# DoubangoTelecom/compv

Measured on AMD Instinct MI355X. Metric: Mpixels/s Sobel->Canny->HoughSHT on 4K uint8, higher is better.
Workload: dtype u8; 1 GPU; batched 3840x2160 uint8 frames, Sobel3x3 -> Canny(59,119) -> HoughSHT(rho=1, theta=1deg, thr=100); 256 distinct frames resident per GPU as 8 batches of 32, a step processes one batch, steps rotate over the batches; frames_per_gpu=32, resident_batches=8, parallelism=frames sharded across 1 GPU(s), no data-path collective

## Files before the change

### compv_amd/csrc/api.cpp

```cpp
#include "api_internal.hpp"

namespace {
__attribute__((noinline, optnone)) float libmCosf(float x) { return cosf(x); }
__attribute__((noinline, optnone)) float libmSinf(float x) { return sinf(x); }

void gradientThresholds(float fLow, float fHigh, int* tLow, int* tHigh)
{
	const float l = fLow < 1.f ? 1.f : (fLow > 65535.f ? 65535.f : fLow);
	const float h = fHigh < 1.f ? 1.f : (fHigh > 65535.f ? 65535.f : fHigh);
	uint16_t lo = static_cast<uint16_t>(l), hi = static_cast<uint16_t>(h);
	lo = static_cast<uint16_t>(std::max<int>(1, lo));
	hi = static_cast<uint16_t>(std::max<int>(lo + 2, hi));
	*tLow = lo; *tHigh = hi;
}

void cannyCoverage(size_t W, int* simdEnd, int* cStart)
{
	const size_t maxCols = W - 1;
	size_t mpw = 1;
	if (maxCols >= 16) mpw = 16; else if (maxCols >= 8) mpw = 8;
	if (mpw == 1) { *simdEnd = 1; *cStart = 1; return; }
	size_t col = 1;
	while (col + (mpw - 1) < maxCols) col += mpw;
	*simdEnd = static_cast<int>(col);
// ... 218 lines not shown
	HIPCHK(ctx, dmalloc(ctx, &p->sinQ, T));
	HIPCHK(ctx, dmalloc(ctx, &p->cosQ, T));
	HIPCHK(ctx, hipMemcpy(p->sinQ, s.data(), T * sizeof(int32_t), hipMemcpyHostToDevice));
	HIPCHK(ctx, hipMemcpy(p->cosQ, c.data(), T * sizeof(int32_t), hipMemcpyHostToDevice));
	{
		std::vector<float> ct(T), ist(T);
		for (size_t t = 0; t < T; ++t) {
			const float theta = static_cast<float>(t) * step;
			ct[t] = libmCosf(theta);
			ist[t] = 1.f / libmSinf(theta);
		}
		HIPCHK(ctx, dmalloc(ctx, &p->cosT, T));
		HIPCHK(ctx, dmalloc(ctx, &p->invSinT, T));
		HIPCHK(ctx, hipMemcpy(p->cosT, ct.data(), T * sizeof(float), hipMemcpyHostToDevice));
		HIPCHK(ctx, hipMemcpy(p->invSinT, ist.data(), T * sizeof(float), hipMemcpyHostToDevice));
	}
	{
		if (p->vt.tiles <= 0 || p->vtKt.size() != static_cast<size_t>(p->vt.tiles) * T) return fail(ctx, COMPVHIP_E_INVALID_STATE, "vote tiles were not planned");
		dfree(ctx, p->dKt); dfree(ctx, p->dRowBase); dfree(ctx, p->partLo); dfree(ctx, p->partHi); dfree(ctx, p->colFlag);
		{
			const int tiles = p->vt.tiles, Rw = p->vt.Rw, groups = sht_nms_groups(static_cast<int>(T));
			std::vector<int2> range(static_cast<size_t>(groups));
			for (int g = 0; g < groups; ++g) {
				int lo = INT32_MAX, hi = INT32_MIN;
				for (int c = 8 * g - 1; c <= 8 * g + 8; ++c) {
					if (c < 0 || c >= static_cast<int>(T)) continue;
					for (int i = 0; i < tiles; ++i) {
						const int b = p->vtRowBase[static_cast<size_t>(i) * T + c];
						lo = std::min(lo, b); hi = std::max(hi, b + Rw);
					}
				}
				range[g] = make_int2(lo - 1, hi + 1);
			}
			std::vector<int2> reach(T);
			for (size_t t = 0; t < T; ++t) {
				int lo = INT32_MAX, hi = INT32_MIN;
				for (int i = 0; i < tiles; ++i) {
					const int b = p->vtRowBase[static_cast<size_t>(i) * T + t];
					lo = std::min(lo, b); hi = std::max(hi, b + Rw);
				}
				reach[t] = make_int2(lo, hi);
			}
			dfree(ctx, p->reach);
			HIPCHK(ctx, dmalloc(ctx, &p->reach, reach.size()));
			HIPCHK(ctx, hipMemcpy(p->reach, reach.data(), reach.size() * sizeof(int2), hipMemcpyHostToDevice));
			dfree(ctx, p->nmsRange);
			HIPCHK(ctx, dmalloc(ctx, &p->nmsRange, range.size()));
			HIPCHK(ctx, hipMemcpy(p->nmsRange, range.data(), range.size() * sizeof(int2), hipMemcpyHostToDevice));
		}
		HIPCHK(ctx, dmalloc(ctx, &p->dKt, p->vtKt.size()));
		HIPCHK(ctx, dmalloc(ctx, &p->dRowBase, p->vtRowBase.size()));
		HIPCHK(ctx, hipMemcpy(p->dKt, p->vtKt.data(), p->vtKt.size() * sizeof(int32_t), hipMemcpyHostToDevice));
		HIPCHK(ctx, hipMemcpy(p->dRowBase, p->vtRowBase.data(), p->vtRowBase.size() * sizeof(int32_t), hipMemcpyHostToDevice));
		{
			const size_t cols = p->frames * p->vt.tiles * static_cast<size_t>(p->vt.Tpad);
			HIPCHK(ctx, dmalloc(ctx, &p->partLo, cols * p->vt.rwPitch));
			HIPCHK(ctx, dmalloc(ctx, &p->partHi, cols * p->vt.rwPitch));
			HIPCHK(ctx, dmalloc(ctx, &p->colFlag, cols));
		}
		p->vt.kt = p->dKt; p->vt.rowBase = p->dRowBase; p->vt.partLo = p->partLo; p->vt.partHi = p->partHi; p->vt.colFlag = p->colFlag; p->vt.reach = p->reach; p->vt.tileCounts = p->tileCounts;
		p->edgeCap = static_cast<size_t>(p->vt.tiles) * p->vt.tileCap;
	}
	HIPCHK(ctx, dmalloc(ctx, &p->edges, p->edgeCap * p->frames));
	HIPCHK(ctx, dmalloc(ctx, &p->acc, p->accFrameStride * p->frames));
	HIPCHK(ctx, hipMemset(p->acc, 0, sizeof(uint16_t) * p->accFrameStride * p->frames));
	p->strengthBits = 1;
	while ((static_cast<size_t>(1) << p->strengthBits) <= 2 * (p->W > p->H ? p->W : p->H)) p->strengthBits++;
	if (p->strengthBits > 16) p->strengthBits = 16;
	int frameBits = 0;
	while ((static_cast<size_t>(1) << frameBits) < p->frames) frameBits++;
	p->keyBits = frameBits + p->strengthBits;
	if (R * T >= (static_cast<size_t>(1) << 32)) return fail(ctx, COMPVHIP_E_INVALID_PARAMETER, "theta step too small: the accumulator has 2^32 cells or more");
	if (p->keyBits > 32) return fail(ctx, COMPVHIP_E_INVALID_PARAMETER, "too many frames for a 32-bit line key");
	dfree(ctx, p->nmsFlags);
	{
		const size_t frows = sht_nms_rows(static_cast<int>(R)), fgroups = static_cast<size_t>(sht_nms_groups(static_cast<int>(T)));
		HIPCHK(ctx, dmalloc(ctx, &p->nmsFlags, frows * fgroups * p->frames));
		HIPCHK(ctx, hipMemset(p->nmsFlags, 0, frows * fgroups * p->frames));
		if (sht_lines_blocks(static_cast<int>(R)) != p->lineBlocks) return fail(ctx, COMPVHIP_E_INVALID_STATE, "row-block counters were sized for another accumulator");
	}
	p->shtReady = true;
	return COMPVHIP_OK;
}

int compvhip_api::ensureLineCap(compvhip_plan* p, size_t cap)
{
	compvhip_ctx* ctx = p->ctx;
	cap = std::min(cap, p->R * p->T);
	if (cap <= p->lineCap) return COMPVHIP_OK;
	dfree(ctx, p->keysA); dfree(ctx, p->keysB); dfree(ctx, p->valsA); dfree(ctx, p->valsB); dfree(ctx, p->sortTemp); dfree(ctx, p->chunkHist); dfree(ctx, p->strengthStart);
	p->lineCap = 0; p->deviceSort = false;
	HIPCHK(ctx, dmalloc(ctx, &p->keysA, cap * p->frames));
	HIPCHK(ctx, dmalloc(ctx, &p->keysB, cap * p->frames));
// ... 183 lines not shown
		if (dmalloc(ctx, &p->sums, frames * kFrameSlot) != hipSuccess) { rc = COMPVHIP_E_OUT_OF_MEMORY; break; }
		if (hipHostMalloc(reinterpret_cast<void**>(&p->hFlags), sizeof(int) * 2 * (kAsyncDepth + 1)) != hipSuccess) { rc = COMPVHIP_E_OUT_OF_MEMORY; break; }
		p->hTotals = reinterpret_cast<unsigned int*>(p->hFlags + kAsyncDepth + 1);
		if (hipHostMalloc(reinterpret_cast<void**>(&p->hRounds), sizeof(int) * (kFrameSlot + 4) * kAsyncDepth, hipHostMallocMapped) != hipSuccess) { rc = COMPVHIP_E_OUT_OF_MEMORY; break; }
		if (hipHostGetDevicePointer(reinterpret_cast<void**>(&p->hRoundsDev), p->hRounds, 0) != hipSuccess) { rc = COMPVHIP_E_HIP; break; }
	} while (0);
	if (rc) { compvhip_plan_destroy(p); return fail(ctx, rc, "plan allocation"); }
	*out = p;
	return COMPVHIP_OK;
}

void compvhip_plan_destroy(compvhip_plan* p)
{
	if (!p) return;
	compvhip_ctx* ctx = p->ctx;
	(void)hipSetDevice(ctx->device);
	timelineClear(p);
	for (hipEvent_t e : p->eventPool) (void)hipEventDestroy(e);
	for (auto& stp : p->steps) if (stp.done) (void)hipEventDestroy(stp.done);
	dfree(ctx, p->dirty);
	dfree(ctx, p->ebits); dfree(ctx, p->ubits); dfree(ctx, p->counters); dfree(ctx, p->thrDev); dfree(ctx, p->sums); dfree(ctx, p->tmpOut);
	if (p->hFlags) (void)hipHostFree(p->hFlags);
	if (p->hRounds) (void)hipHostFree(p->hRounds);
	dfree(ctx, p->hist); dfree(ctx, p->otsu); dfree(ctx, p->blurTmp); dfree(ctx, p->grayTmp);
	dfree(ctx, p->morphTmp);
	dfree(ctx, p->fastWork); dfree(ctx, p->fastScores);
	p->orbIndex.release(ctx); dfree(ctx, p->orbBlur);
	for (KhtBatchState* b : p->khtBatch) khtBatchFree(ctx, b);
	p->khtBatch.clear();
	dfree(ctx, p->cosT); dfree(ctx, p->invSinT);
	dfree(ctx, p->dKt); dfree(ctx, p->dRowBase); dfree(ctx, p->partLo); dfree(ctx, p->partHi); dfree(ctx, p->colFlag);
	dfree(ctx, p->sinQ); dfree(ctx, p->cosQ); dfree(ctx, p->edges); dfree(ctx, p->acc);
	dfree(ctx, p->keysA); dfree(ctx, p->keysB); dfree(ctx, p->valsA); dfree(ctx, p->valsB); dfree(ctx, p->nmsFlags); dfree(ctx, p->chunkHist); dfree(ctx, p->strengthStart);
	dfree(ctx, p->nmsRange); dfree(ctx, p->reach); dfree(ctx, p->sortTemp); p->segPerLine.release(ctx);
	dfree(ctx, p->compRows); dfree(ctx, p->compBits); dfree(ctx, p->compParent);
	delete p;
}

int compvhip_plan_set_timing(compvhip_plan* p, int enabled)
{
	if (!p) return COMPVHIP_E_INVALID_PARAMETER;
	p->timing = (enabled >= 2 && enabled <= 4) ? enabled : (enabled != 0 ? 1 : 0);
	return COMPVHIP_OK;
}

int compvhip_plan_get_timing(compvhip_plan* p, const char** names, float* ms, int cap)
{
	if (!p) return COMPVHIP_E_INVALID_PARAMETER;
	(void)hipSetDevice(p->ctx->device);
	if (!p->timeline.empty()) {
		for (auto& t : p->timeline) (void)hipEventSynchronize(t.b);
		timelineCollect(p);
	}
	const int n = std::min<int>(cap, static_cast<int>(p->timingMs.size()));
	for (int i = 0; i < n; ++i) { if (names) names[i] = p->timingNames[i].c_str(); if (ms) ms[i] = p->timingMs[i]; }
	return n;
}

static int planCannyImpl(compvhip_plan* p, const uint8_t* d_in, float tLow, float tHigh, int ksize, int type, uint8_t* d_edges, hipStream_t st,
                         bool waitConverged, bool clearTimeline = true)
{
	compvhip_ctx* ctx = p->ctx;
	if (!d_in || !d_edges) return fail(ctx, COMPVHIP_E_INVALID_PARAMETER, "null frame pointer");
	int lo, hi;
	int rc = validateCannyParams(ctx, tLow, tHigh, ksize, type, &lo, &hi);
	if (rc) return rc;
	HIPCHK(ctx, hipSetDevice(ctx->device));
// ... 435 lines not shown
```

### compv_amd/csrc/api_internal.hpp

```cpp
#pragma once
#include "../../include/compv_hip.h"
#include "kernels.hpp"
#include "kht.hpp"

#include <hip/hip_runtime.h>

#include <algorithm>
#include <atomic>
#include <chrono>
#include <cmath>
#include <cstdio>
#include <cstdlib>
#include <cstring>
#include <functional>
#include <memory>
#include <string>
#include <thread>
#include <vector>

using namespace compvhip;

namespace compvhip_api {
void countLive(compvhip_ctx* ctx, long delta);

// ... 147 lines not shown
	compvhip_ctx* ctx = nullptr;
	size_t W = 0, H = 0, S = 0, frames = 0;
	float thetaDeg = 1.f;
	int tilesX = 0, tilesY = 0, wb = 0;
	size_t bitsFrameStride = 0;
	uint32_t* ebits = nullptr; uint32_t* ubits = nullptr;
	int* counters = nullptr;
	size_t nCounts = 0;
	int* flags = nullptr; int* hFlags = nullptr;
	int* frameTotals = nullptr; unsigned int* lineTotal = nullptr;
	unsigned int* hTotals = nullptr;
	unsigned int recentTotals[8] = {}; int recentN = 0;
	int specRounds = kSpecRounds; unsigned char recentRounds[8] = {}; int recentRoundsN = 0;
	int* hRoundsDev = nullptr; int* stepHostSlot = nullptr;
	int* hRounds = nullptr;
	int roundsUsed = 0;
	int maxRounds = kMaxRounds;
	bool countersFresh = false;
	int2* thrDev = nullptr; unsigned int* sums = nullptr;
	uint8_t* dirty = nullptr;
	uint8_t* patchOut = nullptr; uint8_t* copyBack = nullptr;
	uint8_t* grayTmp = nullptr;
	uint8_t* tmpOut = nullptr;
	bool bitsValid = false;
	bool shtReady = false;
	size_t R = 0, T = 0; float thetaStep = 0.f; int accPitch = 0;
	uint8_t* blurTmp = nullptr;
	uint32_t* hist = nullptr; int32_t* otsu = nullptr;
	float* cosT = nullptr; float* invSinT = nullptr;
	int32_t* sinQ = nullptr; int32_t* cosQ = nullptr;
	uint32_t* edges = nullptr; size_t edgeCap = 0; int* edgeCounts = nullptr;
	uint16_t* acc = nullptr; size_t accFrameStride = 0;
	uint32_t* keysA = nullptr; uint32_t* keysB = nullptr; uint32_t* valsA = nullptr; uint32_t* valsB = nullptr; size_t lineCap = 0; int* lineCounts = nullptr;
	int2* reach = nullptr;
	int2* nmsRange = nullptr;
	uint8_t* nmsFlags = nullptr;
	int* blockCounts = nullptr; int lineBlocks = 0;
	void* sortTemp = nullptr; size_t sortTempBytes = 0;
	DevBuf<int32_t> segPerLine;
	int32_t* compRows = nullptr; uint32_t* compBits = nullptr; int32_t* compParent = nullptr;
	uint8_t* morphTmp = nullptr;
	int* fastWork = nullptr; uint8_t* fastScores = nullptr;
	DevBuf<int32_t> orbIndex; uint8_t* orbBlur = nullptr; uint16_t orbKern[5] = {}; bool orbKernReady = false; bool orbBriefLds = false;
	int strengthBits = 16, keyBits = 0;
	uint16_t* chunkHist = nullptr; uint32_t* strengthStart = nullptr; int sortChunks = 0; bool deviceSort = false;
	bool voteTiles = false;
	ShtTileArgs vt = {};
	std::vector<int32_t> vtKt, vtRowBase;
	int32_t* dKt = nullptr; int32_t* dRowBase = nullptr; uint8_t* partLo = nullptr; uint8_t* partHi = nullptr; uint8_t* colFlag = nullptr; int* tileCounts = nullptr;
	std::vector<KhtBatchState*> khtBatch;
	std::vector<std::unique_ptr<KhtPeaksWork>> khtWork;
	double khtStageMs[6] = {}; double khtWallMs = 0.0; int khtThreads = 0;
	struct AsyncStep { bool used = false; bool replay = false; uint64_t seq = 0; hipEvent_t done = nullptr; hipStream_t stream = nullptr; StepParams sp; size_t sortN = 0; int rounds = 0; } steps[kAsyncDepth];
	uint64_t stepSeq = 0;
};

struct compvhip_matcher : TimingState {
	compvhip_ctx* ctx = nullptr;
	int descDwords = 0, queryCap = 0, trainCap = 0, pairs = 0, knn = 0;
	uint32_t* partial = nullptr;
	compvhip_match* reverse = nullptr;
};
namespace compvhip_api {

inline void countLive(compvhip_ctx* ctx, long delta) { ctx->live += delta; }

inline int fail(compvhip_ctx* ctx, int code, const char* what, hipError_t e = hipSuccess)
// ... 90 lines not shown
```

### compv_amd/csrc/kernels.hpp

```cpp
#pragma once
#include <hip/hip_runtime.h>
#include <stddef.h>
#include <stdint.h>

#include "../../include/compv_hip.h"

namespace compvhip {

#ifndef COMPVHIP_BAND_H
#define COMPVHIP_BAND_H 64
#endif
constexpr int kBandH = COMPVHIP_BAND_H;
#ifndef COMPVHIP_BAND_WORDS
#define COMPVHIP_BAND_WORDS 64
#endif
constexpr int kBandWords = COMPVHIP_BAND_WORDS;
constexpr int kResolveThreads = 512;
constexpr int kFrameSlot = 32;
constexpr int kResolveRows = kBandH * kBandWords / kResolveThreads;

struct CannyArgs {
	const uint8_t* in;
	uint8_t* out;
	uint32_t* ebits;
// ... 74 lines not shown
	uint32_t* edges;
	int* edgeCounts;
	uint16_t* acc;
	const int32_t* sinQ;
	const int32_t* cosQ;
	uint32_t* lineKeys;
	uint32_t* lineVals;
	uint8_t* nmsFlags;
	int nmsRows;
	int* blockCounts;
	int lineBlocks;
	const int2* nmsRange;
	int nmsGroups;
	int* lineCounts;
	const int* stepFlags;
	int* hostStep;
	int32_t* outCounts;
	int* frameTotals;
	unsigned int* lineTotal;
	size_t sortN;
	size_t bitsFrameStride, edgeCap, accFrameStride, lineCap;
	int W, H, wb;
	int R, T, accPitch, barrier;
	int threshold, nmsLastCol;
	int frames;
	int strengthBits;
};
struct ShtTileArgs {
	const int32_t* kt;
	const int32_t* rowBase;
	uint8_t* partLo;
	uint8_t* partHi;
	uint8_t* colFlag;
	const int2* reach;
	int* tileCounts;
	int nx, ny, TW, TH, tiles;
	int Rw, rwPitch;
	int Tpad, groups;
	size_t tileCap;
};
constexpr int kShtMaxWindow = 1264;
hipError_t launch_sht_compact_tiles(const ShtArgs& a, const ShtTileArgs& v, int frames, hipStream_t stream);
hipError_t launch_sht_vote_tiles(const ShtArgs& a, const ShtTileArgs& v, int frames, hipStream_t stream);
hipError_t launch_sht_reduce_tiles(const ShtArgs& a, const ShtTileArgs& v, int frames, hipStream_t stream);
hipError_t launch_bytes_to_bits(const uint8_t* edges, int W, int H, int S, size_t frameStride, uint32_t* ebits, int wb, size_t bitsFrameStride,
                                int frames, hipStream_t stream);
hipError_t launch_sht_lines(const ShtArgs& a, int frames, hipStream_t stream);
hipError_t launch_sht_decode(const uint32_t* keys, const uint32_t* vals, const int* counts, size_t lineCap, int frames, int T, int barrier, float thetaStep,
                             int maxLines, int strengthBits, void* lines , size_t outCap, hipStream_t stream);
int sht_nms_groups(int T);
size_t sht_nms_rows(int R);
int sht_lines_blocks(int R);
hipError_t launch_sht_cartesian(const void* lines , const int* counts, size_t lineCap, int maxLines, int frames, int T, const float* cosT,
                                const float* invSinT, float thetaStep, float widthF, float r, float* out , hipStream_t stream);
hipError_t launch_sht_acc_transpose(const uint16_t* accT, int R, int T, int accPitch, int32_t* out, size_t outStride, hipStream_t stream);
constexpr int kShtSortChunk = 4096;
constexpr int kShtSortMaxStrengthBits = 13;
constexpr int kShtSortMaxChunks = 32;
struct ShtSortArgs {
	uint32_t* sortedKeys;
	uint32_t* sortedVals;
	uint16_t* chunkHist;
	uint32_t* strengthStart;
	int chunks;
};
hipError_t launch_sht_sort_lines(const ShtArgs& a, const ShtSortArgs& q, int frames, float thetaStep, int maxLines, void* lines , size_t outCap,
                                 hipStream_t stream);
// ... 171 lines not shown
```

### compv_amd/csrc/sht_sort_kernels.hip

```cpp
#include "device.hpp"

#include <type_traits>

namespace compvhip {

namespace {

constexpr int kChunk = kShtSortChunk;
constexpr int kSortThreads = 1024;
constexpr int kBins = 1 << kShtSortMaxStrengthBits;
static_assert(kChunk == 4096 && kBins == 8192, "key layout: 13 bits of inverted strength above 12 bits of chunk position");

}

__global__ __launch_bounds__(kSortThreads) void sht_chunk_sort_kernel(ShtArgs a, ShtSortArgs q)
{
	__shared__ uint32_t s_key[kChunk];
	__shared__ uint32_t s_hist[kBins];
	__shared__ uint32_t s_cnt[kSortThreads], s_wsum[kSortThreads / 64];
	__shared__ unsigned long long s_part[kSortThreads / 64];
	const int frame = blockIdx.y, chunk = blockIdx.x, t = threadIdx.x;
	const size_t nf = min((size_t)max(a.lineCounts[frame], 0), a.lineCap);
	const size_t c0 = (size_t)chunk * kChunk;
	if (c0 >= nf) return;
	const int m = (int)min((size_t)kChunk, nf - c0);
	const size_t base = dense_frame_base<kSortThreads>(a.lineCounts, frame, a.lineCap, s_part) + c0;
	const uint32_t mask = (1u << a.strengthBits) - 1u;
	const uint32_t* __restrict__ kin = a.lineKeys + base;
	const uint32_t* __restrict__ vin = a.lineVals + base;
	uint32_t e[4];
	{
		uint32_t kraw[4];
#pragma unroll
		for (int u = 0; u < 4; ++u) kraw[u] = kin[min(u * kSortThreads + t, m - 1)];
		asm volatile("" : "+v"(kraw[0]), "+v"(kraw[1]), "+v"(kraw[2]), "+v"(kraw[3]));
#pragma unroll
		for (int u = 0; u < 4; ++u) {
			const int i = u * kSortThreads + t;
			e[u] = i < m ? (((mask - (kraw[u] & mask)) << 12) | (uint32_t)i) : 0xffffffffu;
		}
	}
#pragma unroll
	for (int u = 0; u < kBins / kSortThreads; ++u) s_hist[t + u * kSortThreads] = 0u;
	const int lane = t & 63, wave = t >> 6;
	auto radix_pass = [&](auto nbits, int shift) {
		constexpr int NB = decltype(nbits)::value, BINS = 1 << NB;
		s_cnt[t] = 0u;
		__syncthreads();
		uint32_t rank[4], slot[4];
#pragma unroll
		for (int u = 0; u < 4; ++u) {
			const uint32_t d = (e[u] >> shift) & (uint32_t)(BINS - 1);
			uint64_t same = ~0ull;
#pragma unroll
			for (int b = 0; b < NB; ++b) {
				const bool bit = (d >> b) & 1u;
				const uint64_t bal = __ballot(bit);
				same &= bit ? bal : ~bal;
			}
			rank[u] = __builtin_amdgcn_mbcnt_hi((uint32_t)(same >> 32), __builtin_amdgcn_mbcnt_lo((uint32_t)same, 0u));
			slot[u] = (d * 4u + (uint32_t)u) * (uint32_t)(kSortThreads / 64) + (uint32_t)wave;
			if (rank[u] == 0u) s_cnt[slot[u]] = (uint32_t)__popcll(same);
		}
		__syncthreads();
		const uint32_t c = s_cnt[t];
		const uint32_t incl = wave_incl_scan(c, lane);
		if (lane == 63) s_wsum[wave] = incl;
		__syncthreads();
		uint32_t before = 0;
#pragma unroll
		for (int w = 0; w < kSortThreads / 64; ++w) before += (w < wave) ? s_wsum[w] : 0u;
		s_cnt[t] = before + incl - c;
		__syncthreads();
#pragma unroll
		for (int u = 0; u < 4; ++u) s_key[s_cnt[slot[u]] + rank[u]] = e[u];
		__syncthreads();
#pragma unroll
		for (int u = 0; u < 4; ++u) e[u] = s_key[u * kSortThreads + t];
	};
	radix_pass(std::integral_constant<int, 4>{}, 12);
	radix_pass(std::integral_constant<int, 3>{}, 16);
	radix_pass(std::integral_constant<int, 3>{}, 19);
	radix_pass(std::integral_constant<int, 3>{}, 22);
	uint32_t* __restrict__ kout = q.sortedKeys + base;
	uint32_t* __restrict__ vout = q.sortedVals + base;
	{
		uint32_t kk[4]; int lo[4], hi[4];
#pragma unroll
		for (int u = 0; u < 4; ++u) { const int i = min(t + u * kSortThreads, m - 1); kk[u] = s_key[i]; lo[u] = 0; hi[u] = i; }
#pragma unroll
		for (int s = 0; s < 12; ++s) {
#pragma unroll
			for (int u = 0; u < 4; ++u) {
				const int mid = (lo[u] + hi[u]) >> 1;
				const bool ge = s_key[mid] >= (kk[u] & ~4095u);
				hi[u] = ge ? mid : hi[u];
				lo[u] = ge ? lo[u] : mid + 1;
			}
		}
		uint32_t cell[4];
#pragma unroll
		for (int u = 0; u < 4; ++u) cell[u] = vin[kk[u] & 4095u];
		asm volatile("" : "+v"(cell[0]), "+v"(cell[1]), "+v"(cell[2]), "+v"(cell[3]));
#pragma unroll
		for (int u = 0; u < 4; ++u) {
			const int i = t + u * kSortThreads;
			if (i < m) {
				kout[i] = (kk[u] & ~4095u) | (uint32_t)(i - lo[u]);
				vout[i] = cell[u];
				atomicAdd(&s_hist[kk[u] >> 12], 1u);
			}
		}
	}
	__syncthreads();
	uint4* __restrict__ hout = reinterpret_cast<uint4*>(q.chunkHist + ((size_t)frame * q.chunks + chunk) * kBins);
	{
// ... 95 lines not shown
```

### compv_amd/csrc/sht_tiles_kernels.hip

```cpp
#include "device.hpp"

namespace compvhip {

constexpr int kTcThreads = 256;
constexpr int kTcRows = 64;
constexpr int kTcStage = 6144;

__global__ __launch_bounds__(kTcThreads) void sht_compact_tiles_kernel(ShtArgs a, ShtTileArgs v)
{
	__shared__ int s_wave[kTcThreads / 64];
	__shared__ int s_base;
	__shared__ uint32_t s_stage[kTcStage];
	const int frame = blockIdx.y;
	const int chunksPerTile = (v.TH + kTcRows - 1) / kTcRows;
	const int tile = blockIdx.x / chunksPerTile, chunk = blockIdx.x - tile * chunksPerTile;
	const int ty = tile / v.nx, tx = tile - ty * v.nx;
	const int x0 = tx * v.TW, y0 = ty * v.TH;
	const int wpr = v.TW >> 5;
	const uint32_t wprInv = (1u << 20) / (uint32_t)wpr + 1u;
	const int ly0 = chunk * kTcRows;
	const int rows = min(min(kTcRows, v.TH - ly0), a.H - (y0 + ly0));
	const int nwords = max(rows, 0) * wpr;
	const uint32_t* __restrict__ bits = a.ebits + (size_t)frame * a.bitsFrameStride;
	const int w0 = x0 >> 5;
	constexpr int kPer = (kTcRows * 40 + kTcThreads - 1) / kTcThreads;
	uint32_t wv[kPer]; int wl[kPer];
	int cnt = 0;
	if (nwords == 0) return;
#pragma unroll
	for (int k = 0; k < kPer; ++k) {
		const int i = min((int)threadIdx.x + k * kTcThreads, nwords - 1);
		const int r = (int)(((uint32_t)i * wprInv) >> 20), c = i - r * wpr;
		wv[k] = bits[(size_t)(y0 + ly0 + r) * a.wb + min(w0 + c, a.wb - 1)];
// ... 29 lines not shown
			uint32_t b = wv[k];
			while (b) {
				const int bit = __ffs(b) - 1;
				b &= b - 1;
				s_stage[lp++] = (uint32_t)(wl[k] + bit);
			}
		}
		__syncthreads();
		const size_t room = (size_t)s_base < v.tileCap ? v.tileCap - (size_t)s_base : 0;
		const int nout = (int)min((size_t)total, room);
		for (int i = threadIdx.x; i < nout; i += kTcThreads) dst[(size_t)s_base + i] = s_stage[i];
		return;
	}
	size_t pos = (size_t)s_base + first;
#pragma unroll
	for (int k = 0; k < kPer; ++k) {
		uint32_t b = wv[k];
		while (b) {
			const int bit = __ffs(b) - 1;
			b &= b - 1;
			if (pos < v.tileCap) dst[pos] = (uint32_t)(wl[k] + bit);
			++pos;
		}
	}
}

constexpr int kVtThreads = 1024;
constexpr int kVtUnroll = 32;

__global__ __launch_bounds__(kVtThreads) void sht_vote_tiles_kernel(ShtArgs a, ShtTileArgs v)
{
	extern __shared__ __attribute__((aligned(16))) uint32_t hist[];
	const int units = a.frames * v.tiles;
	const int xcd = blockIdx.x & 7, k = blockIdx.x >> 3;
	const int g = k % v.groups;
	const int unit = (k / v.groups) * 8 + xcd;
	if (unit >= units) return;
	const int frame = unit / v.tiles, tile = unit - frame * v.tiles;
	const int tid = threadIdx.x, lane = tid & 63;
	const int wave = __builtin_amdgcn_readfirstlane(tid >> 6);

	const int nAll = v.tileCounts[unit];
	if (g == 0 && threadIdx.x == 0 && nAll) atomicAdd(&a.edgeCounts[frame], nAll);
	const int n = min(nAll, (int)v.tileCap);
	const int words = v.Rw * 32;
	uint32_t* const s_any = hist + words;
	if (tid < 2) s_any[tid] = 0u;
	for (int i = tid * 4; i < words; i += kVtThreads * 4) *reinterpret_cast<uint4*>(&hist[i]) = make_uint4(0, 0, 0, 0);

	const int t = g * 64 + lane;
	const int tt = min(t, a.T - 1);
	const int nc = -a.cosQ[tt], ns = -a.sinQ[tt];
	const int K = v.kt[(size_t)tile * a.T + tt];
	uint32_t inc = (t < a.T) ? ((lane & 32) ? 0x10000u : 1u) : 0u;
	asm volatile("" : "+v"(inc));
	const uint32_t lane4 = (uint32_t)(lane & 31) * 4u;
	__syncthreads();

	const uint32_t* __restrict__ list = a.edges + (size_t)unit * v.tileCap;
	typedef uint32_t u32x16 __attribute__((ext_vector_type(16)));
	auto vote = [&](uint32_t e) {
		const int lx = (int)(e & 0xffffu), ly = (int)(e >> 16);
		int val, ad;
		asm volatile("v_mad_i32_i24 %0, %1, %2, %3" : "=v"(val) : "s"(lx), "v"(nc), "v"(K));
		asm volatile("v_mad_i32_i24 %0, %1, %2, %3" : "=v"(val) : "s"(ly), "v"(ns), "v"(val));
		const uint32_t row = (uint32_t)val >> 16;
		asm volatile("v_lshl_add_u32 %0, %1, 7, %2" : "=v"(ad) : "v"(row), "v"(lane4));
		asm volatile("ds_add_u32 %0, %1" : : "v"(ad), "v"(inc) : "memory");
	};
	const int nblk = n / kVtUnroll;
	constexpr int kStep = kVtThreads / 64;
	u32x16 a0, a1, b0, b1;
#define VT_LOAD(r0, r1, blk) asm volatile("s_load_dwordx16 %0, %2, 0x0\n\ts_load_dwordx16 %1, %2, 0x40" : "=&s"(r0), "=&s"(r1) : "s"(list + (size_t)(blk) * kVtUnroll) : "memory")
#define VT_WAIT(r0, r1) asm volatile("s_waitcnt lgkmcnt(0)" : "+s"(r0), "+s"(r1) : : "memory")
#define VT_VOTE(r0, r1) _Pragma("unroll") for (int u = 0; u < 16; ++u) vote(r0[u]); _Pragma("unroll") for (int u = 0; u < 16; ++u) vote(r1[u])
	int b = wave;
	if (b < nblk) {
		VT_LOAD(a0, a1, b);
		VT_WAIT(a0, a1);
		for (;;) {
			const int bn = b + kStep;
			if (bn < nblk) VT_LOAD(b0, b1, bn);
			VT_VOTE(a0, a1);
			if (bn >= nblk) break;
			VT_WAIT(b0, b1);
			b = bn + kStep;
			if (b < nblk) VT_LOAD(a0, a1, b);
			VT_VOTE(b0, b1);
			if (b >= nblk) break;
			VT_WAIT(a0, a1);
		}
	}
#undef VT_LOAD
#undef VT_WAIT
#undef VT_VOTE
	for (int i = nblk * kVtUnroll + wave; i < n; i += kStep) vote(__builtin_amdgcn_readfirstlane(list[i]));
	__builtin_amdgcn_s_waitcnt(0xc07f);
	__syncthreads();

	const size_t column = ((size_t)unit * v.Tpad) + (size_t)g * 64 + lane;
	uint8_t* __restrict__ partLo = v.partLo + column * v.rwPitch;
	uint8_t* __restrict__ partHi = v.partHi + column * v.rwPitch;
	const uint32_t sel1 = (lane & 32) ? 0x07030602u : 0x05010400u;
	typedef uint32_t u32x4 __attribute__((ext_vector_type(4)));
	auto bytes16 = [&](int w0, u32x4& lo, u32x4& hi) {
		uint32_t h[16];
#pragma unroll
		for (int j = 0; j < 16; ++j) h[j] = hist[(w0 + j) * 32 + (lane & 31)];
#pragma unroll
		for (int q = 0; q < 4; ++q) {
			const uint32_t p01 = __builtin_amdgcn_perm(h[4 * q + 1], h[4 * q], sel1), p23 = __builtin_amdgcn_perm(h[4 * q + 3], h[4 * q + 2], sel1);
			lo[q] = __builtin_amdgcn_perm(p23, p01, 0x05040100u);
			hi[q] = __builtin_amdgcn_perm(p23, p01, 0x07060302u);
		}
	};
	uint32_t any = 0u;
	for (int wb = wave * 128; wb < v.Rw; wb += (kVtThreads / 64) * 128)
	for (int w0 = wb; w0 < min(wb + 128, v.Rw); w0 += 16) {
		u32x4 lo, hi;
		bytes16(w0, lo, hi);
		any |= hi.x | hi.y | hi.z | hi.w;
		uint8_t* const dst = partLo + w0;
		asm volatile("global_store_dwordx4 %0, %1, off" : : "v"(dst), "v"(lo) : "memory");
	}
	const uint64_t mine = __ballot(any != 0u);
	if (lane == 0 && mine) { atomicOr(&s_any[0], (uint32_t)mine); atomicOr(&s_any[1], (uint32_t)(mine >> 32)); }
	__syncthreads();
	const uint32_t m0 = s_any[0], m1 = s_any[1];
	const bool flagged = (((lane & 32) ? m1 : m0) >> (lane & 31)) & 1u;
	if (wave == 0) v.colFlag[column] = flagged ? 1 : 0;
	if ((m0 | m1) == 0u) return;
	if (flagged) {
		for (int wb = wave * 128; wb < v.Rw; wb += (kVtThreads / 64) * 128)
		for (int w0 = wb; w0 < min(wb + 128, v.Rw); w0 += 16) {
			u32x4 lo, hi;
			bytes16(w0, lo, hi);
			uint8_t* const dst = partHi + w0;
			asm volatile("global_store_dwordx4 %0, %1, off" : : "v"(dst), "v"(hi) : "memory");
		}
	}
}

constexpr int kRdThreads = 64;
constexpr int kRdRows = 16;

__global__ __launch_bounds__(kRdThreads) void sht_reduce_tiles_kernel(ShtArgs a, ShtTileArgs v)
{
	const int frame = blockIdx.z, theta = blockIdx.y;
	const int2 reach = v.reach[theta];
	if ((int)(blockIdx.x * kRdThreads * kRdRows) >= reach.y || (int)((blockIdx.x + 1) * kRdThreads * kRdRows) <= reach.x) return;
	const int r0 = (blockIdx.x * kRdThreads + threadIdx.x) * kRdRows;
	if (r0 >= a.accPitch) return;
	uint32_t E[4] = { 0, 0, 0, 0 }, O[4] = { 0, 0, 0, 0 };
	int covers = 0;
	for (int tile = 0; tile < v.tiles; ++tile) {
		const int base = v.rowBase[(size_t)tile * a.T + theta];
		const int w0 = r0 - base;
		if (w0 < 0 || w0 >= v.Rw) continue;
		++covers;
		const size_t column = ((size_t)frame * v.tiles + tile) * v.Tpad + theta;
		const uint4 c = *reinterpret_cast<const uint4*>(v.partLo + column * v.rwPitch + w0);
		E[0] += c.x & 0x00ff00ffu; O[0] += (c.x >> 8) & 0x00ff00ffu;
		E[1] += c.y & 0x00ff00ffu; O[1] += (c.y >> 8) & 0x00ff00ffu;
		E[2] += c.z & 0x00ff00ffu; O[2] += (c.z >> 8) & 0x00ff00ffu;
		E[3] += c.w & 0x00ff00ffu; O[3] += (c.w >> 8) & 0x00ff00ffu;
		if (v.colFlag[column]) {
			const uint4 h = *reinterpret_cast<const uint4*>(v.partHi + column * v.rwPitch + w0);
			E[0] += (h.x & 0x00ff00ffu) << 8; O[0] += h.x & 0xff00ff00u;
			E[1] += (h.y & 0x00ff00ffu) << 8; O[1] += h.y & 0xff00ff00u;
			E[2] += (h.z & 0x00ff00ffu) << 8; O[2] += h.z & 0xff00ff00u;
			E[3] += (h.w & 0x00ff00ffu) << 8; O[3] += h.w & 0xff00ff00u;
		}
	}
	if (!covers) return;
	uint32_t o[8];
#pragma unroll
	for (int d = 0; d < 4; ++d) {
		o[2 * d] = (E[d] & 0xffffu) | (O[d] << 16);
		o[2 * d + 1] = (E[d] >> 16) | (O[d] & 0xffff0000u);
	}
	uint4* dst = reinterpret_cast<uint4*>(a.acc + (size_t)frame * a.accFrameStride + (size_t)theta * a.accPitch + r0);
	dst[0] = make_uint4(o[0], o[1], o[2], o[3]);
	dst[1] = make_uint4(o[4], o[5], o[6], o[7]);
}

hipError_t launch_sht_compact_tiles(const ShtArgs& a, const ShtTileArgs& v, int frames, hipStream_t stream)
{
	const int chunksPerTile = (v.TH + kTcRows - 1) / kTcRows;
	dim3 grid((unsigned)(v.tiles * chunksPerTile), frames);
	hipLaunchKernelGGL(sht_compact_tiles_kernel, grid, dim3(kTcThreads), 0, stream, a, v);
	return hipGetLastError();
}

size_t sht_vote_tiles_lds_bytes(int Rw) { return (size_t)Rw * 128 + 16; }

hipError_t launch_sht_vote_tiles(const ShtArgs& a, const ShtTileArgs& v, int frames, hipStream_t stream)
{
	const size_t lds = sht_vote_tiles_lds_bytes(v.Rw);
	if (lds > 160 * 1024) return hipErrorInvalidValue;
	static size_t attr_lds[64] = {};
	int dev = 0;
	(void)hipGetDevice(&dev);
	dev = (dev >= 0 && dev < 64) ? dev : 0;
	if (lds > attr_lds[dev]) {
		hipError_t e = hipFuncSetAttribute(reinterpret_cast<const void*>(sht_vote_tiles_kernel), hipFuncAttributeMaxDynamicSharedMemorySize, (int)lds);
		if (e != hipSuccess) return e;
		attr_lds[dev] = lds;
	}
	const int units = frames * v.tiles;
	dim3 grid((unsigned)(8 * ((units + 7) / 8) * v.groups));
	hipLaunchKernelGGL(sht_vote_tiles_kernel, grid, dim3(kVtThreads), lds, stream, a, v);
	return hipGetLastError();
}

hipError_t launch_sht_reduce_tiles(const ShtArgs& a, const ShtTileArgs& v, int frames, hipStream_t stream)
{
	dim3 grid((unsigned)((a.R + kRdThreads * kRdRows - 1) / (kRdThreads * kRdRows)), a.T, frames);
	hipLaunchKernelGGL(sht_reduce_tiles_kernel, grid, dim3(kRdThreads), 0, stream, a, v);
	return hipGetLastError();
}

}
```

Baseline: 424,200 Mpixels/s.

## Persist vote blocks, precompute reduce work lists, skip constant radix passes

New measurement: 421,600 Mpixels/s. Within noise of the previous version (-0.6%).

```diff
diff --git a/compv_amd/csrc/api.cpp b/compv_amd/csrc/api.cpp
--- a/compv_amd/csrc/api.cpp
+++ b/compv_amd/csrc/api.cpp
@@ -274,18 +274,24 @@
 				}
 				range[g] = make_int2(lo - 1, hi + 1);
 			}
-			std::vector<int2> reach(T);
-			for (size_t t = 0; t < T; ++t) {
-				int lo = INT32_MAX, hi = INT32_MIN;
+			const int blockRows = 1024, nblocks = (p->accPitch + blockRows - 1) / blockRows;
+			std::vector<int4> blocks;
+			std::vector<int2> covering;
+			for (size_t t = 0; t < T; ++t) for (int b = 0; b < nblocks; ++b) {
+				const int first = static_cast<int>(covering.size());
 				for (int i = 0; i < tiles; ++i) {
-					const int b = p->vtRowBase[static_cast<size_t>(i) * T + t];
-					lo = std::min(lo, b); hi = std::max(hi, b + Rw);
+					const int base = p->vtRowBase[static_cast<size_t>(i) * T + t];
+					if (base < (b + 1) * blockRows && base + Rw > b * blockRows) covering.push_back(make_int2(i, base));
 				}
-				reach[t] = make_int2(lo, hi);
+				const int n = static_cast<int>(covering.size()) - first;
+				if (n) blocks.push_back(make_int4(static_cast<int>(t), b, first, n));
 			}
-			dfree(ctx, p->reach);
-			HIPCHK(ctx, dmalloc(ctx, &p->reach, reach.size()));
-			HIPCHK(ctx, hipMemcpy(p->reach, reach.data(), reach.size() * sizeof(int2), hipMemcpyHostToDevice));
+			dfree(ctx, p->rdBlocks); dfree(ctx, p->rdTiles);
+			p->vt.rdLive = static_cast<int>(blocks.size());
+			HIPCHK(ctx, dmalloc(ctx, &p->rdBlocks, std::max<size_t>(blocks.size(), 1)));
+			HIPCHK(ctx, dmalloc(ctx, &p->rdTiles, std::max<size_t>(covering.size(), 1)));
+			HIPCHK(ctx, hipMemcpy(p->rdBlocks, blocks.data(), blocks.size() * sizeof(int4), hipMemcpyHostToDevice));
+			HIPCHK(ctx, hipMemcpy(p->rdTiles, covering.data(), covering.size() * sizeof(int2), hipMemcpyHostToDevice));
 			dfree(ctx, p->nmsRange);
 			HIPCHK(ctx, dmalloc(ctx, &p->nmsRange, range.size()));
 			HIPCHK(ctx, hipMemcpy(p->nmsRange, range.data(), range.size() * sizeof(int2), hipMemcpyHostToDevice));
@@ -299,8 +305,9 @@
 			HIPCHK(ctx, dmalloc(ctx, &p->partLo, cols * p->vt.rwPitch));
 			HIPCHK(ctx, dmalloc(ctx, &p->partHi, cols * p->vt.rwPitch));
 			HIPCHK(ctx, dmalloc(ctx, &p->colFlag, cols));
+			HIPCHK(ctx, hipMemset(p->colFlag, 0, cols));
 		}
-		p->vt.kt = p->dKt; p->vt.rowBase = p->dRowBase; p->vt.partLo = p->partLo; p->vt.partHi = p->partHi; p->vt.colFlag = p->colFlag; p->vt.reach = p->reach; p->vt.tileCounts = p->tileCounts;
+		p->vt.kt = p->dKt; p->vt.rowBase = p->dRowBase; p->vt.partLo = p->partLo; p->vt.partHi = p->partHi; p->vt.colFlag = p->colFlag; p->vt.rdBlocks = p->rdBlocks; p->vt.rdTiles = p->rdTiles; p->vt.tileCounts = p->tileCounts;
 		p->edgeCap = static_cast<size_t>(p->vt.tiles) * p->vt.tileCap;
 	}
 	HIPCHK(ctx, dmalloc(ctx, &p->edges, p->edgeCap * p->frames));
@@ -550,7 +557,7 @@
 	dfree(ctx, p->dKt); dfree(ctx, p->dRowBase); dfree(ctx, p->partLo); dfree(ctx, p->partHi); dfree(ctx, p->colFlag);
 	dfree(ctx, p->sinQ); dfree(ctx, p->cosQ); dfree(ctx, p->edges); dfree(ctx, p->acc);
 	dfree(ctx, p->keysA); dfree(ctx, p->keysB); dfree(ctx, p->valsA); dfree(ctx, p->valsB); dfree(ctx, p->nmsFlags); dfree(ctx, p->chunkHist); dfree(ctx, p->strengthStart);
-	dfree(ctx, p->nmsRange); dfree(ctx, p->reach); dfree(ctx, p->sortTemp); p->segPerLine.release(ctx);
+	dfree(ctx, p->nmsRange); dfree(ctx, p->rdBlocks); dfree(ctx, p->rdTiles); dfree(ctx, p->sortTemp); p->segPerLine.release(ctx);
 	dfree(ctx, p->compRows); dfree(ctx, p->compBits); dfree(ctx, p->compParent);
 	delete p;
 }
diff --git a/compv_amd/csrc/api_internal.hpp b/compv_amd/csrc/api_internal.hpp
--- a/compv_amd/csrc/api_internal.hpp
+++ b/compv_amd/csrc/api_internal.hpp
@@ -203,7 +203,7 @@
 	uint32_t* edges = nullptr; size_t edgeCap = 0; int* edgeCounts = nullptr;
 	uint16_t* acc = nullptr; size_t accFrameStride = 0;
 	uint32_t* keysA = nullptr; uint32_t* keysB = nullptr; uint32_t* valsA = nullptr; uint32_t* valsB = nullptr; size_t lineCap = 0; int* lineCounts = nullptr;
-	int2* reach = nullptr;
+	int4* rdBlocks = nullptr; int2* rdTiles = nullptr;
 	int2* nmsRange = nullptr;
 	uint8_t* nmsFlags = nullptr;
 	int* blockCounts = nullptr; int lineBlocks = 0;
diff --git a/compv_amd/csrc/kernels.hpp b/compv_amd/csrc/kernels.hpp
--- a/compv_amd/csrc/kernels.hpp
+++ b/compv_amd/csrc/kernels.hpp
@@ -130,7 +130,9 @@
 	uint8_t* partLo;
 	uint8_t* partHi;
 	uint8_t* colFlag;
-	const int2* reach;
+	const int4* rdBlocks;
+	const int2* rdTiles;
+	int rdLive;
 	int* tileCounts;
 	int nx, ny, TW, TH, tiles;
 	int Rw, rwPitch;
diff --git a/compv_amd/csrc/sht_sort_kernels.hip b/compv_amd/csrc/sht_sort_kernels.hip
--- a/compv_amd/csrc/sht_sort_kernels.hip
+++ b/compv_amd/csrc/sht_sort_kernels.hip
@@ -19,11 +19,13 @@
 	__shared__ uint32_t s_hist[kBins];
 	__shared__ uint32_t s_cnt[kSortThreads], s_wsum[kSortThreads / 64];
 	__shared__ unsigned long long s_part[kSortThreads / 64];
+	__shared__ uint32_t s_bits[2];
 	const int frame = blockIdx.y, chunk = blockIdx.x, t = threadIdx.x;
 	const size_t nf = min((size_t)max(a.lineCounts[frame], 0), a.lineCap);
 	const size_t c0 = (size_t)chunk * kChunk;
 	if (c0 >= nf) return;
 	const int m = (int)min((size_t)kChunk, nf - c0);
+	if (t == 0) { s_bits[0] = 0u; s_bits[1] = ~0u; }
 	const size_t base = dense_frame_base<kSortThreads>(a.lineCounts, frame, a.lineCap, s_part) + c0;
 	const uint32_t mask = (1u << a.strengthBits) - 1u;
 	const uint32_t* __restrict__ kin = a.lineKeys + base;
@@ -43,6 +45,20 @@
 #pragma unroll
 	for (int u = 0; u < kBins / kSortThreads; ++u) s_hist[t + u * kSortThreads] = 0u;
 	const int lane = t & 63, wave = t >> 6;
+	{
+		uint32_t vo = 0u, va = ~0u;
+#pragma unroll
+		for (int u = 0; u < 4; ++u) {
+			const bool valid = u * kSortThreads + t < m;
+			vo |= valid ? e[u] >> 12 : 0u;
+			va &= valid ? e[u] >> 12 : ~0u;
+		}
+#pragma unroll
+		for (int o = 32; o > 0; o >>= 1) { vo |= __shfl_xor(vo, o); va &= __shfl_xor(va, o); }
+		if (lane == 0) { atomicOr(&s_bits[0], vo); atomicAnd(&s_bits[1], va); }
+	}
+	__syncthreads();
+	const uint32_t differ = (s_bits[0] ^ s_bits[1]) << 12;
 	auto radix_pass = [&](auto nbits, int shift) {
 		constexpr int NB = decltype(nbits)::value, BINS = 1 << NB;
 		s_cnt[t] = 0u;
@@ -78,10 +94,15 @@
 #pragma unroll
 		for (int u = 0; u < 4; ++u) e[u] = s_key[u * kSortThreads + t];
 	};
-	radix_pass(std::integral_constant<int, 4>{}, 12);
-	radix_pass(std::integral_constant<int, 3>{}, 16);
-	radix_pass(std::integral_constant<int, 3>{}, 19);
-	radix_pass(std::integral_constant<int, 3>{}, 22);
+	if (differ & (15u << 12)) radix_pass(std::integral_constant<int, 4>{}, 12);
+	if (differ & (7u << 16)) radix_pass(std::integral_constant<int, 3>{}, 16);
+	if (differ & (7u << 19)) radix_pass(std::integral_constant<int, 3>{}, 19);
+	if (differ & (7u << 22)) radix_pass(std::integral_constant<int, 3>{}, 22);
+	if (!(differ & (0x1fffu << 12))) {
+#pragma unroll
+		for (int u = 0; u < 4; ++u) s_key[u * kSortThreads + t] = e[u];
+		__syncthreads();
+	}
 	uint32_t* __restrict__ kout = q.sortedKeys + base;
 	uint32_t* __restrict__ vout = q.sortedVals + base;
 	{
diff --git a/compv_amd/csrc/sht_tiles_kernels.hip b/compv_amd/csrc/sht_tiles_kernels.hip
--- a/compv_amd/csrc/sht_tiles_kernels.hip
+++ b/compv_amd/csrc/sht_tiles_kernels.hip
@@ -1,4 +1,6 @@
 #include "device.hpp"
+
+#include <algorithm>
 
 namespace compvhip {
 
@@ -94,113 +96,150 @@
 {
 	extern __shared__ __attribute__((aligned(16))) uint32_t hist[];
 	const int units = a.frames * v.tiles;
-	const int xcd = blockIdx.x & 7, k = blockIdx.x >> 3;
-	const int g = k % v.groups;
-	const int unit = (k / v.groups) * 8 + xcd;
-	if (unit >= units) return;
-	const int frame = unit / v.tiles, tile = unit - frame * v.tiles;
+	const int xcd = blockIdx.x & 7;
+	const int kEnd = ((units + 7) >> 3) * v.groups, kStride = (int)(gridDim.x >> 3);
 	const int tid = threadIdx.x, lane = tid & 63;
 	const int wave = __builtin_amdgcn_readfirstlane(tid >> 6);
-
-	const int nAll = v.tileCounts[unit];
-	if (g == 0 && threadIdx.x == 0 && nAll) atomicAdd(&a.edgeCounts[frame], nAll);
-	const int n = min(nAll, (int)v.tileCap);
+	auto unitOf = [&](int k) { return (k / v.groups) * 8 + xcd; };
+	auto nextItem = [&](int k) { while (k < kEnd && unitOf(k) >= units) k += kStride; return k; };
+	int k = nextItem((int)(blockIdx.x >> 3));
+	if (k >= kEnd) return;
+
 	const int words = v.Rw * 32;
 	uint32_t* const s_any = hist + words;
 	if (tid < 2) s_any[tid] = 0u;
 	for (int i = tid * 4; i < words; i += kVtThreads * 4) *reinterpret_cast<uint4*>(&hist[i]) = make_uint4(0, 0, 0, 0);
-
-	const int t = g * 64 + lane;
-	const int tt = min(t, a.T - 1);
-	const int nc = -a.cosQ[tt], ns = -a.sinQ[tt];
-	const int K = v.kt[(size_t)tile * a.T + tt];
-	uint32_t inc = (t < a.T) ? ((lane & 32) ? 0x10000u : 1u) : 0u;
-	asm volatile("" : "+v"(inc));
 	const uint32_t lane4 = (uint32_t)(lane & 31) * 4u;
+	const uint32_t sel1 = (lane & 32) ? 0x07030602u : 0x05010400u;
+	constexpr int kStep = kVtThreads / 64;
+
+	typedef uint32_t u32x16 __attribute__((ext_vector_type(16)));
+	typedef uint32_t u32x4 __attribute__((ext_vector_type(4)));
+	u32x16 a0, a1, b0, b1;
+#define VT_LOAD(r0, r1, ptr) asm volatile("s_load_dwordx16 %0, %2, 0x0\n\ts_load_dwordx16 %1, %2, 0x40" : "=&s"(r0), "=&s"(r1) : "s"(ptr) : "memory")
+#define VT_WAIT(r0, r1) asm volatile("s_waitcnt lgkmcnt(0)" : "+s"(r0), "+s"(r1) : : "memory")
+#define VT_LOAD_FIRST(ptr) asm volatile("s_load_dwordx16 %0, %2, 0x0\n\ts_load_dwordx16 %1, %2, 0x40" : "=&{s[36:51]}"(a0), "=&{s[52:67]}"(a1) : "s"(ptr) : "memory")
+#define VT_WAIT_FIRST() asm volatile("s_waitcnt lgkmcnt(0)" : "+{s[36:51]}"(a0), "+{s[52:67]}"(a1) : : "memory")
+#define VT_VOTE(r0, r1) _Pragma("unroll") for (int u = 0; u < 16; ++u) vote(r0[u]); _Pragma("unroll") for (int u = 0; u < 16; ++u) vote(r1[u])
+
+	auto thetaOf = [&](int kk) { return (kk % v.groups) * 64 + lane; };
+	int nAll = v.tileCounts[unitOf(k)];
+	int K, nc, ns;
+	{
+		const int tt = min(thetaOf(k), a.T - 1);
+		nc = -a.cosQ[tt]; ns = -a.sinQ[tt];
+		K = v.kt[(size_t)(unitOf(k) % v.tiles) * a.T + tt];
+	}
+	if (wave < min(nAll, (int)v.tileCap) / kVtUnroll) VT_LOAD_FIRST(a.edges + (size_t)unitOf(k) * v.tileCap + (size_t)wave * kVtUnroll);
 	__syncthreads();
 
-	const uint32_t* __restrict__ list = a.edges + (size_t)unit * v.tileCap;
-	typedef uint32_t u32x16 __attribute__((ext_vector_type(16)));
-	auto vote = [&](uint32_t e) {
-		const int lx = (int)(e & 0xffffu), ly = (int)(e >> 16);
-		int val, ad;
-		asm volatile("v_mad_i32_i24 %0, %1, %2, %3" : "=v"(val) : "s"(lx), "v"(nc), "v"(K));
-		asm volatile("v_mad_i32_i24 %0, %1, %2, %3" : "=v"(val) : "s"(ly), "v"(ns), "v"(val));
-		const uint32_t row = (uint32_t)val >> 16;
-		asm volatile("v_lshl_add_u32 %0, %1, 7, %2" : "=v"(ad) : "v"(row), "v"(lane4));
-		asm volatile("ds_add_u32 %0, %1" : : "v"(ad), "v"(inc) : "memory");
-	};
-	const int nblk = n / kVtUnroll;
-	constexpr int kStep = kVtThreads / 64;
-	u32x16 a0, a1, b0, b1;
-#define VT_LOAD(r0, r1, blk) asm volatile("s_load_dwordx16 %0, %2, 0x0\n\ts_load_dwordx16 %1, %2, 0x40" : "=&s"(r0), "=&s"(r1) : "s"(list + (size_t)(blk) * kVtUnroll) : "memory")
-#define VT_WAIT(r0, r1) asm volatile("s_waitcnt lgkmcnt(0)" : "+s"(r0), "+s"(r1) : : "memory")
-#define VT_VOTE(r0, r1) _Pragma("unroll") for (int u = 0; u < 16; ++u) vote(r0[u]); _Pragma("unroll") for (int u = 0; u < 16; ++u) vote(r1[u])
-	int b = wave;
-	if (b < nblk) {
-		VT_LOAD(a0, a1, b);
-		VT_WAIT(a0, a1);
-		for (;;) {
-			const int bn = b + kStep;
-			if (bn < nblk) VT_LOAD(b0, b1, bn);
-			VT_VOTE(a0, a1);
-			if (bn >= nblk) break;
-			VT_WAIT(b0, b1);
-			b = bn + kStep;
-			if (b < nblk) VT_LOAD(a0, a1, b);
-			VT_VOTE(b0, b1);
-			if (b >= nblk) break;
-			VT_WAIT(a0, a1);
-		}
+	for (;;) {
+		const int unit = unitOf(k), g = k % v.groups;
+		const int frame = unit / v.tiles;
+		if (g == 0 && threadIdx.x == 0 && nAll) atomicAdd(&a.edgeCounts[frame], nAll);
+		const int n = min(nAll, (int)v.tileCap);
+		const int t = g * 64 + lane;
+		uint32_t inc = (t < a.T) ? ((lane & 32) ? 0x10000u : 1u) : 0u;
+		asm volatile("" : "+v"(inc));
+		const int kNext = nextItem(k + kStride);
+		const bool more = kNext < kEnd;
+		int nAllN = 0, KN = 0, ncN = 0, nsN = 0;
+		if (more) {
+			const int un = unitOf(kNext), tt = min(thetaOf(kNext), a.T - 1);
+			nAllN = v.tileCounts[un];
+			ncN = -a.cosQ[tt]; nsN = -a.sinQ[tt];
+			KN = v.kt[(size_t)(un % v.tiles) * a.T + tt];
+		}
+
+		const uint32_t* __restrict__ list = a.edges + (size_t)unit * v.tileCap;
+		auto vote = [&](uint32_t e) {
+			const int lx = (int)(e & 0xffffu), ly = (int)(e >> 16);
+			int val, ad;
+			asm volatile("v_mad_i32_i24 %0, %1, %2, %3" : "=v"(val) : "s"(lx), "v"(nc), "v"(K));
+			asm volatile("v_mad_i32_i24 %0, %1, %2, %3" : "=v"(val) : "s"(ly), "v"(ns), "v"(val));
+			const uint32_t row = (uint32_t)val >> 16;
+			asm volatile("v_lshl_add_u32 %0, %1, 7, %2" : "=v"(ad) : "v"(row), "v"(lane4));
+			asm volatile("ds_add_u32 %0, %1" : : "v"(ad), "v"(inc) : "memory");
+		};
+		const int nblk = n / kVtUnroll;
+		int b = wave;
+		if (b < nblk) {
+			VT_WAIT_FIRST();
+			for (;;) {
+				const int bn = b + kStep;
+				if (bn < nblk) VT_LOAD(b0, b1, list + (size_t)bn * kVtUnroll);
+				VT_VOTE(a0, a1);
+				if (bn >= nblk) break;
+				VT_WAIT(b0, b1);
+				b = bn + kStep;
+				if (b < nblk) VT_LOAD(a0, a1, list + (size_t)b * kVtUnroll);
+				VT_VOTE(b0, b1);
+				if (b >= nblk) break;
+				VT_WAIT(a0, a1);
+			}
+		}
+		for (int i = nblk * kVtUnroll + wave; i < n; i += kStep) vote(__builtin_amdgcn_readfirstlane(list[i]));
+		asm volatile("" : : "v"(KN), "v"(ncN), "v"(nsN), "s"(nAllN));
+		__builtin_amdgcn_s_waitcnt(0xc07f);
+		__syncthreads();
+
+		if (more && wave < min(nAllN, (int)v.tileCap) / kVtUnroll) VT_LOAD_FIRST(a.edges + (size_t)unitOf(kNext) * v.tileCap + (size_t)wave * kVtUnroll);
+
+		const bool owns = t < a.T;
+		const size_t column = ((size_t)unit * v.Tpad) + (size_t)g * 64 + lane;
+		uint8_t* __restrict__ partLo = v.partLo + column * v.rwPitch;
+		uint8_t* __restrict__ partHi = v.partHi + column * v.rwPitch;
+		auto bytes16 = [&](int w0, u32x4& lo, u32x4& hi) {
+			uint32_t h[16];
+#pragma unroll
+			for (int j = 0; j < 16; ++j) h[j] = hist[(w0 + j) * 32 + (lane & 31)];
+#pragma unroll
+			for (int q = 0; q < 4; ++q) {
+				const uint32_t p01 = __builtin_amdgcn_perm(h[4 * q + 1], h[4 * q], sel1), p23 = __builtin_amdgcn_perm(h[4 * q + 3], h[4 * q + 2], sel1);
+				lo[q] = __builtin_amdgcn_perm(p23, p01, 0x05040100u);
+				hi[q] = __builtin_amdgcn_perm(p23, p01, 0x07060302u);
+			}
+		};
+		uint32_t any = 0u;
+		if (owns) {
+			for (int wb = wave * 128; wb < v.Rw; wb += (kVtThreads / 64) * 128)
+			for (int w0 = wb; w0 < min(wb + 128, v.Rw); w0 += 16) {
+				u32x4 lo, hi;
+				bytes16(w0, lo, hi);
+				any |= hi.x | hi.y | hi.z | hi.w;
+				uint8_t* const dst = partLo + w0;
+				asm volatile("global_store_dwordx4 %0, %1, off" : : "v"(dst), "v"(lo) : "memory");
+			}
+		}
+		const uint64_t mine = __ballot(any != 0u);
+		if (lane == 0 && mine) { atomicOr(&s_any[0], (uint32_t)mine); atomicOr(&s_any[1], (uint32_t)(mine >> 32)); }
+		__syncthreads();
+		const uint32_t m0 = s_any[0], m1 = s_any[1];
+		const bool flagged = (((lane & 32) ? m1 : m0) >> (lane & 31)) & 1u;
+		if (wave == 0 && owns) v.colFlag[column] = flagged ? 1 : 0;
+		if ((m0 | m1) != 0u && flagged) {
+			for (int wb = wave * 128; wb < v.Rw; wb += (kVtThreads / 64) * 128)
+			for (int w0 = wb; w0 < min(wb + 128, v.Rw); w0 += 16) {
+				u32x4 lo, hi;
+				bytes16(w0, lo, hi);
+				uint8_t* const dst = partHi + w0;
+				asm volatile("global_store_dwordx4 %0, %1, off" : : "v"(dst), "v"(hi) : "memory");
+			}
+		}
+		if (!more) return;
+		for (int wb = wave * 128; wb < v.Rw; wb += (kVtThreads / 64) * 128) {
+			const int end = min(wb + 128, v.Rw) * 32;
+			for (int i = wb * 32 + lane * 4; i < end; i += 64 * 4) *reinterpret_cast<uint4*>(&hist[i]) = make_uint4(0, 0, 0, 0);
+		}
+		__syncthreads();
+		if (tid < 2) s_any[tid] = 0u;
+		k = kNext; nAll = nAllN; K = KN; nc = ncN; ns = nsN;
 	}
 #undef VT_LOAD
 #undef VT_WAIT
+#undef VT_LOAD_FIRST
+#undef VT_WAIT_FIRST
 #undef VT_VOTE
-	for (int i = nblk * kVtUnroll + wave; i < n; i += kStep) vote(__builtin_amdgcn_readfirstlane(list[i]));
-	__builtin_amdgcn_s_waitcnt(0xc07f);
-	__syncthreads();
-
-	const size_t column = ((size_t)unit * v.Tpad) + (size_t)g * 64 + lane;
-	uint8_t* __restrict__ partLo = v.partLo + column * v.rwPitch;
-	uint8_t* __restrict__ partHi = v.partHi + column * v.rwPitch;
-	const uint32_t sel1 = (lane & 32) ? 0x07030602u : 0x05010400u;
-	typedef uint32_t u32x4 __attribute__((ext_vector_type(4)));
-	auto bytes16 = [&](int w0, u32x4& lo, u32x4& hi) {
-		uint32_t h[16];
-#pragma unroll
-		for (int j = 0; j < 16; ++j) h[j] = hist[(w0 + j) * 32 + (lane & 31)];
-#pragma unroll
-		for (int q = 0; q < 4; ++q) {
-			const uint32_t p01 = __builtin_amdgcn_perm(h[4 * q + 1], h[4 * q], sel1), p23 = __builtin_amdgcn_perm(h[4 * q + 3], h[4 * q + 2], sel1);
-			lo[q] = __builtin_amdgcn_perm(p23, p01, 0x05040100u);
-			hi[q] = __builtin_amdgcn_perm(p23, p01, 0x07060302u);
-		}
-	};
-	uint32_t any = 0u;
-	for (int wb = wave * 128; wb < v.Rw; wb += (kVtThreads / 64) * 128)
-	for (int w0 = wb; w0 < min(wb + 128, v.Rw); w0 += 16) {
-		u32x4 lo, hi;
-		bytes16(w0, lo, hi);
-		any |= hi.x | hi.y | hi.z | hi.w;
-		uint8_t* const dst = partLo + w0;
-		asm volatile("global_store_dwordx4 %0, %1, off" : : "v"(dst), "v"(lo) : "memory");
-	}
-	const uint64_t mine = __ballot(any != 0u);
-	if (lane == 0 && mine) { atomicOr(&s_any[0], (uint32_t)mine); atomicOr(&s_any[1], (uint32_t)(mine >> 32)); }
-	__syncthreads();
-	const uint32_t m0 = s_any[0], m1 = s_any[1];
-	const bool flagged = (((lane & 32) ? m1 : m0) >> (lane & 31)) & 1u;
-	if (wave == 0) v.colFlag[column] = flagged ? 1 : 0;
-	if ((m0 | m1) == 0u) return;
-	if (flagged) {
-		for (int wb = wave * 128; wb < v.Rw; wb += (kVtThreads / 64) * 128)
-		for (int w0 = wb; w0 < min(wb + 128, v.Rw); w0 += 16) {
-			u32x4 lo, hi;
-			bytes16(w0, lo, hi);
-			uint8_t* const dst = partHi + w0;
-			asm volatile("global_store_dwordx4 %0, %1, off" : : "v"(dst), "v"(hi) : "memory");
-		}
-	}
 }
 
 constexpr int kRdThreads = 64;
@@ -208,31 +247,42 @@
 
 __global__ __launch_bounds__(kRdThreads) void sht_reduce_tiles_kernel(ShtArgs a, ShtTileArgs v)
 {
-	const int frame = blockIdx.z, theta = blockIdx.y;
-	const int2 reach = v.reach[theta];
-	if ((int)(blockIdx.x * kRdThreads * kRdRows) >= reach.y || (int)((blockIdx.x + 1) * kRdThreads * kRdRows) <= reach.x) return;
-	const int r0 = (blockIdx.x * kRdThreads + threadIdx.x) * kRdRows;
+	const int frame = blockIdx.y;
+	const int4 blk = v.rdBlocks[blockIdx.x];
+	const int theta = blk.x;
+	const int r0 = (blk.y * kRdThreads + threadIdx.x) * kRdRows;
 	if (r0 >= a.accPitch) return;
+	const int2* __restrict__ cover = v.rdTiles + blk.z;
+	const int ncover = blk.w;
 	uint32_t E[4] = { 0, 0, 0, 0 }, O[4] = { 0, 0, 0, 0 };
 	int covers = 0;
-	for (int tile = 0; tile < v.tiles; ++tile) {
-		const int base = v.rowBase[(size_t)tile * a.T + theta];
-		const int w0 = r0 - base;
-		if (w0 < 0 || w0 >= v.Rw) continue;
-		++covers;
-		const size_t column = ((size_t)frame * v.tiles + tile) * v.Tpad + theta;
-		const uint4 c = *reinterpret_cast<const uint4*>(v.partLo + column * v.rwPitch + w0);
+	auto addLo = [&](const uint4& c) {
 		E[0] += c.x & 0x00ff00ffu; O[0] += (c.x >> 8) & 0x00ff00ffu;
 		E[1] += c.y & 0x00ff00ffu; O[1] += (c.y >> 8) & 0x00ff00ffu;
 		E[2] += c.z & 0x00ff00ffu; O[2] += (c.z >> 8) & 0x00ff00ffu;
 		E[3] += c.w & 0x00ff00ffu; O[3] += (c.w >> 8) & 0x00ff00ffu;
-		if (v.colFlag[column]) {
-			const uint4 h = *reinterpret_cast<const uint4*>(v.partHi + column * v.rwPitch + w0);
-			E[0] += (h.x & 0x00ff00ffu) << 8; O[0] += h.x & 0xff00ff00u;
-			E[1] += (h.y & 0x00ff00ffu) << 8; O[1] += h.y & 0xff00ff00u;
-			E[2] += (h.z & 0x00ff00ffu) << 8; O[2] += h.z & 0xff00ff00u;
-			E[3] += (h.w & 0x00ff00ffu) << 8; O[3] += h.w & 0xff00ff00u;
-		}
+	};
+	auto addHi = [&](const uint4& h) {
+		E[0] += (h.x & 0x00ff00ffu) << 8; O[0] += h.x & 0xff00ff00u;
+		E[1] += (h.y & 0x00ff00ffu) << 8; O[1] += h.y & 0xff00ff00u;
+		E[2] += (h.z & 0x00ff00ffu) << 8; O[2] += h.z & 0xff00ff00u;
+		E[3] += (h.w & 0x00ff00ffu) << 8; O[3] += h.w & 0xff00ff00u;
+	};
+	const uint4 zero4 = make_uint4(0u, 0u, 0u, 0u);
+	for (int i = 0; i < ncover; i += 2) {
+		const int2 t0 = cover[i], t1 = cover[min(i + 1, ncover - 1)];
+		const int w0 = r0 - t0.y, w1 = r0 - t1.y;
+		const bool in0 = w0 >= 0 && w0 < v.Rw, in1 = i + 1 < ncover && w1 >= 0 && w1 < v.Rw;
+		const size_t col0 = ((size_t)frame * v.tiles + t0.x) * v.Tpad + theta, col1 = ((size_t)frame * v.tiles + t1.x) * v.Tpad + theta;
+		const uint8_t f0 = v.colFlag[col0], f1 = v.colFlag[col1];
+		uint4 c0 = zero4, c1 = zero4;
+		if (in0) c0 = *reinterpret_cast<const uint4*>(v.partLo + col0 * v.rwPitch + w0);
+		if (in1) c1 = *reinterpret_cast<const uint4*>(v.partLo + col1 * v.rwPitch + w1);
+		covers |= (int)in0 | (int)in1;
+		addLo(c0);
+		addLo(c1);
+		if (f0 && in0) addHi(*reinterpret_cast<const uint4*>(v.partHi + col0 * v.rwPitch + w0));
+		if (f1 && in1) addHi(*reinterpret_cast<const uint4*>(v.partHi + col1 * v.rwPitch + w1));
 	}
 	if (!covers) return;
 	uint32_t o[8];
@@ -269,15 +319,25 @@
 		if (e != hipSuccess) return e;
 		attr_lds[dev] = lds;
 	}
+	static int cus[64] = {};
+	if (!cus[dev]) {
+		hipDeviceProp_t prop;
+		hipError_t e = hipGetDeviceProperties(&prop, dev);
+		if (e != hipSuccess) return e;
+		cus[dev] = std::max(8, prop.multiProcessorCount & ~7);
+	}
 	const int units = frames * v.tiles;
-	dim3 grid((unsigned)(8 * ((units + 7) / 8) * v.groups));
+	const int items = 8 * ((units + 7) / 8) * v.groups;
+	dim3 grid((unsigned)std::min(cus[dev], items));
 	hipLaunchKernelGGL(sht_vote_tiles_kernel, grid, dim3(kVtThreads), lds, stream, a, v);
 	return hipGetLastError();
 }
 
 hipError_t launch_sht_reduce_tiles(const ShtArgs& a, const ShtTileArgs& v, int frames, hipStream_t stream)
 {
-	dim3 grid((unsigned)((a.R + kRdThreads * kRdRows - 1) / (kRdThreads * kRdRows)), a.T, frames);
+	static_assert(kRdThreads * kRdRows == 1024, "the row blocks of the plan's work list (ensureSht)");
+	if (v.rdLive <= 0) return hipSuccess;
+	dim3 grid((unsigned)v.rdLive, frames);
 	hipLaunchKernelGGL(sht_reduce_tiles_kernel, grid, dim3(kRdThreads), 0, stream, a, v);
 	return hipGetLastError();
 }
```
